# MAC-VO/MAC-VO

Measured on NVIDIA H100. Metric: stereo frames/sec @640x480, higher is better.
Workload: dtype f32

## Files before the change

### include/macvo_b200.h

```cpp
#ifndef MACVO_B200_H
#define MACVO_B200_H

#include <stddef.h>
#include <stdint.h>

#ifdef __cplusplus
extern "C" {
#endif

#define MACVO_OK 0
#define MACVO_E_ARG (-1)
#define MACVO_E_WORKSPACE (-2)
#define MACVO_E_UNSUPPORTED (-3)
#define MACVO_E_DRIVER (-4)

const char* macvo_b200_version(void);

#define MACVO_CORR_SIMT 0
#define MACVO_CORR_TC_3XF16 1
#define MACVO_CORR_TC_1XF16 2
#define MACVO_CORR_TC_TF32 3
#define MACVO_CORR_KMAJOR_INPUT 16
size_t macvo_corr_workspace_bytes(int batch, int dim, int n, int mode);
int macvo_corr_build(const float* fmap1, const float* fmap2, float* corr, int batch, int dim, int n, int mode,
// ... 88 lines not shown
                            const double* intr, double* pose_io, const macvo_pgo_params_t* params, double* stats,
                            void* const* exchange_bufs, int world, int rank, void* stream);

#define MACVO_PGO_ACC 55
#define MACVO_PGO_MAX_RANKS 8
int macvo_pgo_accumulate(const double* pos_Tw, const double* kp2_uv, const double* kp2_disp, const double* uv_cov,
                         const double* disp_cov, int k, const double* intr, const double* pose, double huber_delta,
                         double* acc, void* stream);

int macvo_layer_norm(const float* x, const float* weight, const float* bias, float* y, long long rows,
                     int channels, float eps, void* stream);
int macvo_add_layer_norm(const float* x, const float* resid, const float* weight, const float* bias, float* sum_out,
                         float* y, long long rows, int channels, float eps, void* stream);
int macvo_mlp_tc(const float* xn, const float* resid, const float* w1, const float* b1, const float* w2, const float* b2,
                 float* out, int rows, int channels, int hidden, void* stream);
int macvo_patch_tokens_tc(const float* x, const float* w0, const float* term, const float* w2, const float* b2,
                          const float* ln_w, const float* ln_b, float* out, long long rows, int in_channels, int channels,
                          int period, float eps, void* stream);
int macvo_patch_embed_conv1(const float* maps, const float* weight, const float* bias, float* out,
                            long long n_maps, int h, int w, int allow_tf32, void* stream);
int macvo_add_rows_relu(float* x, const float* term, long long rows, int period, int channels, void* stream);
int macvo_small_attention(const float* q, const float* k, const float* v, float* out, int batch, int nq, int nk,
                          int heads, int head_dim, int q_broadcast, int allow_tf32, void* stream);

int macvo_small_attention_ex(const float* q, const float* k, const float* v, float* out, int batch, int nq, int nk,
                             int heads, int head_dim, int q_broadcast, int allow_tf32, int ldq, int ldk, int ldv,
                             const float* q_add, const float* k_add, int add_period, void* stream);

int macvo_latent_pool(const float* tokens, const float* ut, const float* wv, const float* bv, float* out,
                      long long n_maps, int nk, void* stream);
// ... 76 lines not shown
```

### mac-vo_b200/csrc/mlp_tc.cu

```cuda
#include "tc_common.cuh"

namespace {

constexpr int MLP_C = 128, MLP_ROWS = 128, MLP_CHUNK = 64;
constexpr int XN_BYTES = MLP_ROWS * MLP_C * 4;
constexpr int XN_SUB = MLP_ROWS * 128;
constexpr int W1_BYTES = MLP_CHUNK * MLP_C * 4;
constexpr int W1_SUB = MLP_CHUNK * 128;
constexpr int W2_BYTES = MLP_C * MLP_CHUNK * 4;
constexpr int W2_SUB = MLP_C * 128;
constexpr int HID_WG_BYTES = 64 * MLP_CHUNK * 4;
constexpr int HID_SUB = 64 * 128;
constexpr int OFF_W1 = XN_BYTES, OFF_W2 = OFF_W1 + 2 * W1_BYTES, OFF_HID = OFF_W2 + 2 * W2_BYTES;
constexpr int OFF_BAR = OFF_HID + 2 * HID_WG_BYTES;
constexpr int MLP_SMEM = OFF_BAR + 128 + 1024;
static_assert(MLP_SMEM <= 227 * 1024, "shared memory budget");

constexpr uint32_t SW128_DESC_HI = (1024u >> 4) | (1u << 30);
__device__ __forceinline__ uint32_t sw128_lo(uint32_t smem_addr) { return ((smem_addr & 0x3FFFFu) >> 4) | (1u << 16); }
__device__ __forceinline__ uint64_t sw128_desc(uint32_t lo) { return ((uint64_t)SW128_DESC_HI << 32) | lo; }

__device__ __forceinline__ uint32_t to_tf32(float x) {
    uint32_t r;
    asm("cvt.rn.tf32.f32 %0, %1;" : "=r"(r) : "f"(x));
    return r;
}

constexpr int MLP_THREADS = TC_CONSUMER_THREADS + 128;

__global__ void __launch_bounds__(MLP_THREADS, 1)
mlp_tc_kernel(const __grid_constant__ CUtensorMap map_x, const __grid_constant__ CUtensorMap map_w1,
              const __grid_constant__ CUtensorMap map_w2, const float* __restrict__ b1, const float* __restrict__ b2,
              const float* __restrict__ resid, float* __restrict__ out, int m, int hd) {
    extern __shared__ uint8_t smem_raw[];
    uint8_t* smem = reinterpret_cast<uint8_t*>((reinterpret_cast<uintptr_t>(smem_raw) + 1023) & ~(uintptr_t)1023);
    const uint32_t s_base = smem_u32(smem);
    const uint32_t bar_x = s_base + OFF_BAR, bar_w1f = bar_x + 8, bar_w1e = bar_w1f + 16, bar_w2f = bar_w1e + 16,
                   bar_w2e = bar_w2f + 16;
    const int warp = threadIdx.x >> 5, lane = threadIdx.x & 31;
    const int m0 = blockIdx.x * MLP_ROWS, chunks = hd / MLP_CHUNK;

    if (threadIdx.x == 0) {
        mbar_init(bar_x, 1);
        for (int s = 0; s < 2; ++s) {
            mbar_init(bar_w1f + 8 * s, 1); mbar_init(bar_w1e + 8 * s, 2);
            mbar_init(bar_w2f + 8 * s, 1); mbar_init(bar_w2e + 8 * s, 2);
        }
        fence_barrier_init();
        prefetch_tmap(&map_x); prefetch_tmap(&map_w1); prefetch_tmap(&map_w2);
    }
    __syncthreads();

    if (warp >= TC_PRODUCER_WARP) {
        asm volatile("setmaxnreg.dec.sync.aligned.u32 40;");
        if (warp == TC_PRODUCER_WARP && elect_one()) {
            mbar_expect_tx(bar_x, XN_BYTES);
            for (int kc = 0; kc < 4; ++kc) tma_load_2d(s_base + kc * XN_SUB, &map_x, bar_x, 32 * kc, m0);
            for (int j = 0; j < chunks; ++j) {
                const int s = j & 1;
                const uint32_t parity = ((j >> 1) & 1) ^ 1;
                mbar_wait(bar_w1e + 8 * s, parity);
                mbar_expect_tx(bar_w1f + 8 * s, W1_BYTES);
                for (int kc = 0; kc < 4; ++kc)
                    tma_load_2d(s_base + OFF_W1 + s * W1_BYTES + kc * W1_SUB, &map_w1, bar_w1f + 8 * s, 32 * kc, j * MLP_CHUNK);
                mbar_wait(bar_w2e + 8 * s, parity);
                mbar_expect_tx(bar_w2f + 8 * s, W2_BYTES);
                for (int h = 0; h < 2; ++h)
                    tma_load_2d(s_base + OFF_W2 + s * W2_BYTES + h * W2_SUB, &map_w2, bar_w2f + 8 * s, j * MLP_CHUNK + 32 * h, 0);
            }
        }
        return;
    }
// ... 34 lines not shown
        if (leader) {
            mbar_arrive(bar_w1e + 8 * (j & 1));
            if (j > 0) mbar_arrive(bar_w2e + 8 * ((j - 1) & 1));
        }
        const float* bj = b1 + j * MLP_CHUNK;
#pragma unroll
        for (int i = 0; i < 32; i += 2) {
            const int r = fr + 8 * ((i >> 1) & 1), c = 8 * (i >> 2) + fc;
            const float2 bb = __ldg(reinterpret_cast<const float2*>(bj + c));
            const uint32_t v0 = to_tf32(gelu_erf(h[i] + bb.x)), v1 = to_tf32(gelu_erf(h[i + 1] + bb.y));
            const int cc = c & 31;
            const uint32_t addr = hid + (c >> 5) * HID_SUB + r * 128 + ((((cc >> 2) ^ (r & 7))) << 4) + (cc & 3) * 4;
            asm volatile("st.shared.v2.b32 [%0], {%1, %2};" ::"r"(addr), "r"(v0), "r"(v1) : "memory");
        }
        asm volatile("fence.proxy.async.shared::cta;" ::: "memory");
        if (wg == 0) asm volatile("bar.sync 2, 128;" ::: "memory");
        else asm volatile("bar.sync 3, 128;" ::: "memory");
        const int s = j & 1;
        mbar_wait(bar_w2f + 8 * s, (j >> 1) & 1);
        uint32_t hd_ = hid_d;
        asm volatile("" : "+r"(hd_));
        const uint32_t wb = hd_ - ((OFF_HID + wg * HID_WG_BYTES) >> 4) + ((OFF_W2 + s * W2_BYTES) >> 4);
        wgmma_fence();
#pragma unroll
        for (int hh = 0; hh < 2; ++hh) {
#pragma unroll
            for (int k = 0; k < 4; ++k)
                Wgmma<128>::tf32(acc, sw128_desc(hd_ + (hh * HID_SUB >> 4) + 2 * k), sw128_desc(wb + (hh * W2_SUB >> 4) + 2 * k),
                                 (j | hh | k) != 0);
        }
        wgmma_commit();
    };

    mbar_wait(bar_x, 0);
    {
        const int t = threadIdx.x & 127;
#pragma unroll
        for (int kc = 0; kc < 4; ++kc) {
#pragma unroll
            for (int u = 0; u < 4; ++u) {
                const uint32_t a = s_base + kc * XN_SUB + wg * 64 * 128 + (u * 128 + t) * 16;
                const float4 v = lds128(a);
                asm volatile("st.shared.v4.b32 [%0], {%1, %2, %3, %4};" ::"r"(a), "r"(to_tf32(v.x)), "r"(to_tf32(v.y)),
                             "r"(to_tf32(v.z)), "r"(to_tf32(v.w)) : "memory");
            }
        }
        asm volatile("fence.proxy.async.shared::cta;" ::: "memory");
        if (wg == 0) asm volatile("bar.sync 2, 128;" ::: "memory");
        else asm volatile("bar.sync 3, 128;" ::: "memory");
    }
    gemm1(h0, 0);
    for (int j = 0; j < chunks; j += 2) {
        chunk(h0, h1, j);
        chunk(h1, h0, j + 1);
    }
    wgmma_wait<0>();
    fence_acc(acc);

    const int row0 = m0 + wg * 64 + fr;
#pragma unroll
    for (int i = 0; i < 64; i += 2) {
        const int r = row0 + 8 * ((i >> 1) & 1), c = 8 * (i >> 2) + fc;
        if (r < m) {
            const float2 bb = __ldg(reinterpret_cast<const float2*>(b2 + c));
            const float2 x = __ldg(reinterpret_cast<const float2*>(resid + (long long)r * MLP_C + c));
            *reinterpret_cast<float2*>(out + (long long)r * MLP_C + c) = make_float2(x.x + (acc[i] + bb.x), x.y + (acc[i + 1] + bb.y));
        }
    }
}

}

int macvo_mlp_tc(const float* xn, const float* resid, const float* w1, const float* b1, const float* w2, const float* b2,
                 float* out, int rows, int channels, int hidden, void* stream) {
    if (!xn || !resid || !w1 || !b1 || !w2 || !b2 || !out || rows <= 0) return MACVO_E_ARG;
    if (channels != MLP_C || (hidden != 128 && hidden != 512)) return MACVO_E_UNSUPPORTED;
    for (const void* p : {(const void*)xn, (const void*)resid, (const void*)w1, (const void*)b1, (const void*)w2,
                          (const void*)b2, (const void*)out})
        if (reinterpret_cast<uintptr_t>(p) & 15) return MACVO_E_ARG;
    CUtensorMap m_x, m_w1, m_w2;
    bool ok = make_map_2d(&m_x, CU_TENSOR_MAP_DATA_TYPE_FLOAT32, 4, xn, MLP_C, rows, MLP_C * 4, 32, MLP_ROWS);
    ok = ok && make_map_2d(&m_w1, CU_TENSOR_MAP_DATA_TYPE_FLOAT32, 4, w1, MLP_C, hidden, MLP_C * 4, 32, MLP_CHUNK);
    ok = ok && make_map_2d(&m_w2, CU_TENSOR_MAP_DATA_TYPE_FLOAT32, 4, w2, hidden, MLP_C, (uint64_t)hidden * 4, 32, MLP_C);
    if (!ok) return MACVO_E_DRIVER;
    static bool configured = false;
    if (!configured) {
        MACVO_CUDA_TRY(cudaFuncSetAttribute(mlp_tc_kernel, cudaFuncAttributeMaxDynamicSharedMemorySize, MLP_SMEM));
        configured = true;
    }
    mlp_tc_kernel<<<ceil_div(rows, MLP_ROWS), MLP_THREADS, MLP_SMEM, as_stream(stream)>>>(m_x, m_w1, m_w2, b1, b2, resid, out,
                                                                                          rows, hidden);
    MACVO_LAUNCH_CHECK();
    return MACVO_OK;
}
```

### mac-vo_b200/flowformer_cov.py

```python
from __future__ import annotations

import math
import os
import zlib
from typing import Callable

import torch
import torch.nn.functional as F

Tensor = torch.Tensor

LATENT_TOKENS = 8
LATENT_DIM = 128
QUERY_DIM = 64
COST_INPUT_DIM = 64
VERT_C_DIM = 64
ENCODER_DEPTH = 3


def _svt_spec(prefix: str) -> list[tuple[str, tuple[int, ...], str]]:
    out: list[tuple[str, tuple[int, ...], str]] = []
    dims, heads, srs, patch, cin = (128, 256), (4, 8), (8, 4), (4, 2), (3, 128)
    for s, (C, sr, ps, ci) in enumerate(zip(dims, srs, patch, cin)):
        p = f"{prefix}.svt."
# ... 272 lines not shown
        return o.permute(0, 2, 1, 3).reshape(B, I, C)

    def _memo(self, key, fn):
        if key not in self._cache:
            self._cache[key] = fn()
        return self._cache[key]

    def svt(self, x: Tensor, prefix: str) -> Tensor:
        B = x.shape[0]
        for s, (heads, sr, ps) in enumerate(((4, 8, 4), (8, 4, 2))):
            p = f"{prefix}.svt."
            x = self._conv(x, p + f"patch_embeds.{s}.proj", stride=ps)
            C, H, W = x.shape[1:]
            x = self._ln(x.flatten(2).transpose(1, 2), p + f"patch_embeds.{s}.norm")
            b0, b1 = p + f"blocks.{s}.0.", p + f"blocks.{s}.1."
            x, xn = self._add_ln(x, self._svt_local_attn(self._ln(x, b0 + "norm1", 1e-6), (H, W), b0 + "attn.", heads), b0 + "norm2", 1e-6)
            x = self._mlp_residual(x, xn, b0 + "mlp.", "fc1", "fc2")
            t = x.transpose(1, 2).reshape(B, C, H, W)
            t = self._conv(t, p + f"pos_block.{s}.proj.0", padding=1, groups=C) + t
            x = t.flatten(2).transpose(1, 2)
            x, xn = self._add_ln(x, self._svt_global_attn(self._ln(x, b1 + "norm1", 1e-6), (H, W), b1 + "attn.", heads, sr), b1 + "norm2", 1e-6)
            x = self._mlp_residual(x, xn, b1 + "mlp.", "fc1", "fc2")
            x = x.reshape(B, H, W, C).permute(0, 3, 1, 2)
        return x

    def _mlp_residual(self, x: Tensor, xn: Tensor, p: str, fc1: str, fc2: str) -> Tensor:
        w1 = self.W[p + fc1 + ".weight"]
        if (self.mlp_tensor_cores and self._native(x) and torch.backends.cuda.matmul.allow_tf32 and x.shape[-1] == 128
                and w1.shape[0] in self._ops.MLP_TC_HIDDEN and x.is_contiguous() and xn.is_contiguous()):
            w1t, w2t = self._memo(("mlp_tc", p), lambda: (self._ops.round_tf32(w1), self._ops.round_tf32(self.W[p + fc2 + ".weight"])))
            return self._ops.mlp_tc(xn, x, w1t, self.W[p + fc1 + ".bias"], w2t, self.W[p + fc2 + ".bias"])
        return x + self._lin(F.gelu(self._lin(xn, p + fc1)), p + fc2)

    @staticmethod
    def _to_windows(x: Tensor, ws: int) -> tuple[Tensor, tuple[int, int, int, int]]:
        B, H, W, C = x.shape
        pr, pb = (ws - W % ws) % ws, (ws - H % ws) % ws
        x = F.pad(x, (0, 0, 0, pr, 0, pb))
        nh, nw = (H + pb) // ws, (W + pr) // ws
        x = x.reshape(B, nh, ws, nw, ws, C).transpose(2, 3).reshape(B * nh * nw, ws * ws, C)
        return x, (B, nh, nw, C)

    @staticmethod
    def _from_windows(x: Tensor, meta: tuple[int, int, int, int], ws: int, H: int, W: int) -> Tensor:
        B, nh, nw, C = meta
        x = x.reshape(B, nh, nw, ws, ws, C).transpose(2, 3).reshape(B, nh * ws, nw * ws, C)
        return x[:, :H, :W, :].reshape(B, H * W, C)

    def _svt_local_attn(self, x: Tensor, size, p: str, heads: int, ws: int = 7) -> Tensor:
        B, N, C = x.shape
        H, W = size
        xw, meta = self._to_windows(x.view(B, H, W, C), ws)
        wq, bq = self.W[p + "qkv.weight"], self.W[p + "qkv.bias"]
        q, k, v = (F.linear(xw, wq[i * C:(i + 1) * C], bq[i * C:(i + 1) * C]) for i in range(3))
        o = self._attn(q, k, v, heads)
        return self._lin(self._from_windows(o, meta, ws, H, W), p + "proj")

    def _svt_global_attn(self, x: Tensor, size, p: str, heads: int, sr: int) -> Tensor:
        B, N, C = x.shape
        q = self._lin(x, p + "q")
        t = self._conv(x.permute(0, 2, 1).reshape(B, C, *size), p + "sr", stride=sr)
        t = self._ln(t.reshape(B, C, -1).permute(0, 2, 1), p + "norm")
        wkv, bkv = self.W[p + "kv.weight"], self.W[p + "kv.bias"]
        o = self._attn(q, F.linear(t, wkv[:C], bkv[:C]), F.linear(t, wkv[C:], bkv[C:]), heads)
        return self._lin(o, p + "proj")

    def patch_embed(self, cost_maps: Tensor) -> Tensor:
        p = "memory_encoder.cost_perceiver_encoder.patch_embed."
        M, _, H2, W2 = cost_maps.shape
        if self._native(cost_maps) and (H2 + 7) // 8 * 8 * ((W2 + 7) // 8 * 8) <= 96 * 160:
            if torch.backends.cudnn.allow_tf32:
                x = self._ops.patch_embed_conv1(cost_maps, self.W[p + "proj.0.weight"], self.W[p + "proj.0.bias"], s2d=True)
                w2 = self._memo(("pe_w2_s2d", x.device), lambda: self._ops.space_to_depth_filter(self.W[p + "proj.2.weight"])
                                .contiguous(memory_format=torch.channels_last))
                x = torch.cudnn_convolution_relu(x, w2, self.W[p + "proj.2.bias"], (1, 1), (1, 1), (1, 1), 1)
            else:
                x = self._ops.patch_embed_conv1(cost_maps, self.W[p + "proj.0.weight"], self.W[p + "proj.0.bias"])
                x = self._conv_relu(x, p + "proj.2", stride=2, padding=2)
        else:
            x = F.pad(cost_maps, (0, (8 - W2 % 8) % 8, 0, (8 - H2 % 8) % 8))
# ... 17 lines not shown
        t = x.permute(0, 2, 3, 1).reshape(M, h * w, COST_INPUT_DIM)
        w2 = self.W[p + "ffn_with_coord.2.weight"][:, :, 0, 0]
        if native and torch.backends.cuda.matmul.allow_tf32:
            w0t, w2t = self._memo(("pe_tc", x.device), lambda: (self._ops.round_tf32(w0[:, :COST_INPUT_DIM, 0, 0]),
                                                                self._ops.round_tf32(w2)))
            return self._ops.patch_tokens_tc(t, w0t, term[0], w2t, self.W[p + "ffn_with_coord.2.bias"],
                                             self.W[p + "norm.weight"], self.W[p + "norm.bias"])
        t = F.linear(t, w0[:, :COST_INPUT_DIM, 0, 0])
        t = self._ops.add_rows_relu_(t, term[0]) if native else F.relu(t + term)
        t = F.linear(t, w2, self.W[p + "ffn_with_coord.2.bias"])
        return self._ln(t, p + "norm")

    def _latent_layer(self, x: Tensor, p: str) -> Tensor:
        y = self._ln(x, p + "norm1")
        a = self._attn(self._lin(y, p + "q"), self._lin(y, p + "k"), self._lin(y, p + "v"), 8)
        x, xn = self._add_ln(x, self._lin(a, p + "proj"), p + "norm2")
        return self._mlp_residual(x, xn, p, "ffn.0", "ffn.3")

    def _context_tokens(self, context: Tensor, p: str, reps: int) -> Tensor:
        b, _, H, W = context.shape
        c = self._lin(context.flatten(2).permute(0, 2, 1), p + "context_proj").view(b, H, W, -1)
        return c.repeat(reps, 1, 1, 1)

    def _vert_local_attn_native(self, x: Tensor, size, context: Tensor, p: str, ws: int, heads: int) -> Tensor:
        Bt, N, C = x.shape
        H, W = size
        b = context.shape[0]
        wq, wk = self.W[p + "q.weight"], self.W[p + "k.weight"]
        enc = self._memo(("win", ws, C + VERT_C_DIM, x.dtype, x.device), lambda: sine_embed(
            coords_grid(1, ws, ws, x.device, x.dtype).view(1, 2, -1).permute(0, 2, 1), C + VERT_C_DIM))
        cproj = self._lin(context.flatten(2).permute(0, 2, 1), p + "context_proj").view(b, H, W, -1)
        cw, meta = self._to_windows(cproj, ws)
        w_qk_c = torch.cat([wq[:, C:], wk[:, C:]], 0)
        w_qk = torch.cat([wq, wk], 0)
        b_qk = torch.cat([self.W[p + "q.bias"], self.W[p + "k.bias"]], 0)
        terms = F.linear(cw, w_qk_c) + F.linear(enc, w_qk, b_qk)
        q_add, k_add = terms[..., :C].contiguous(), terms[..., C:].contiguous()
        w_x = self._memo(("vloc_w", p), lambda: torch.cat([wq[:, :C], wk[:, :C], self.W[p + "v.weight"]], 0).contiguous())
        b_x = self._memo(("vloc_b", p), lambda: torch.cat([torch.zeros(2 * C, device=x.device, dtype=x.dtype), self.W[p + "v.bias"]], 0))
        xw, meta = self._to_windows(x.view(Bt, H, W, C), ws)
        qkv = F.linear(xw, w_x, b_x)
        o = self._ops.fused_qkv_attention(qkv, heads, q_add, k_add)
        return self._lin(self._from_windows(o, meta, ws, H, W), p + "proj")

    def _vert_local_attn(self, x: Tensor, size, context: Tensor, p: str, ws: int = 7, heads: int = 8) -> Tensor:
        if self._native(x) and (x.shape[-1] // heads) in (16, 32):
            return self._vert_local_attn_native(x, size, context, p, ws, heads)
        Bt, N, C = x.shape
        H, W = size
        ctx = self._context_tokens(context, p, Bt // context.shape[0])
        xg = x.view(Bt, H, W, C)
        xw, meta = self._to_windows(xg, ws)
        qkw, _ = self._to_windows(torch.cat([xg, ctx], dim=-1), ws)
        enc = self._memo(("win", ws, C + VERT_C_DIM, x.dtype, x.device), lambda: sine_embed(
            coords_grid(1, ws, ws, x.device, x.dtype).view(1, 2, -1).permute(0, 2, 1), C + VERT_C_DIM))
        qkw = qkw + enc
        o = self._attn(self._lin(qkw, p + "q"), self._lin(qkw, p + "k"), self._lin(xw, p + "v"), heads)
        return self._lin(self._from_windows(o, meta, ws, H, W), p + "proj")

    def _vert_global_attn_native(self, x: Tensor, size, context: Tensor, p: str, sr: int, heads: int) -> Tensor:
        Bt, N, C = x.shape
        H, W = size
        b = context.shape[0]
        Cq = C + VERT_C_DIM
        wq = self.W[p + "q.weight"]
        cproj = self._lin(context.flatten(2).permute(0, 2, 1), p + "context_proj")
        enc_full = self._memo(("full", H, W, Cq, x.dtype, x.device), lambda: sine_embed(
            coords_grid(1, H, W, x.device, x.dtype).view(1, 2, -1).permute(0, 2, 1), Cq))
        q_add = (F.linear(cproj, wq[:, C:]) + F.linear(enc_full, wq, self.W[p + "q.bias"])).contiguous()
        q = F.linear(x, wq[:, :C])
        xg = x.view(Bt, H, W, C).permute(0, 3, 1, 2)
        wsk = self.W[p + "sr_key.weight"]
        wk_x = self._memo(("vglob_wkx", p), lambda: wsk[:, :C].contiguous(memory_format=torch.channels_last))
        wk_c = self._memo(("vglob_wkc", p), lambda: wsk[:, C:].contiguous(memory_format=torch.channels_last))
        k_ctx = F.conv2d(cproj.view(b, H, W, -1).permute(0, 3, 1, 2), wk_c, self.W[p + "sr_key.bias"], stride=sr)
        k_in = F.conv2d(xg, wk_x, None, stride=sr).permute(0, 2, 3, 1)
        M = k_in.shape[1] * k_in.shape[2]
        k_in = (k_in.reshape(Bt // b, b, M, C) + k_ctx.permute(0, 2, 3, 1).reshape(1, b, M, C)).view(Bt, M, C)
        v_in = self._conv(xg, p + "sr_value", stride=sr).reshape(Bt, C, -1).permute(0, 2, 1)
        v_in, k_in = self._ln(v_in, p + "norm"), self._ln(k_in, p + "norm")
        enc_sub = self._memo(("sub", H // sr, W // sr, sr, C, x.dtype, x.device), lambda: sine_embed(
            coords_grid(1, H // sr, W // sr, x.device, x.dtype).view(1, 2, -1).permute(0, 2, 1) * sr, C))
        o = self._ops.attention_with_terms(q, self._lin(k_in + enc_sub, p + "k"), self._lin(v_in, p + "v"), heads, q_add)
        return self._lin(o, p + "proj")

    def _vert_global_attn(self, x: Tensor, size, context: Tensor, p: str, sr: int = 4, heads: int = 8) -> Tensor:
        if self._native(x) and size[0] % sr == 0 and size[1] % sr == 0 and (x.shape[-1] // heads) in (16, 32):
            return self._vert_global_attn_native(x, size, context, p, sr, heads)
        Bt, N, C = x.shape
        H, W = size
        ctx = self._context_tokens(context, p, Bt // context.shape[0])
        xg = x.view(Bt, H, W, C)
        qk = torch.cat([xg, ctx], dim=-1)
        pr, pb = (sr - W % sr) % sr, (sr - H % sr) % sr
        xg, qk = F.pad(xg, (0, 0, 0, pr, 0, pb)), F.pad(qk, (0, 0, 0, pr, 0, pb))
        Hp, Wp = H + pb, W + pr
        Cq = C + VERT_C_DIM
        enc_full = self._memo(("full", Hp, Wp, Cq, x.dtype, x.device), lambda: sine_embed(
            coords_grid(1, Hp, Wp, x.device, x.dtype).view(1, 2, -1).permute(0, 2, 1), Cq))
        q = self._lin(qk.reshape(Bt, Hp * Wp, Cq) + enc_full, p + "q")
        v_in = self._conv(xg.permute(0, 3, 1, 2), p + "sr_value", stride=sr).reshape(Bt, C, -1).permute(0, 2, 1)
        k_in = self._conv(qk.permute(0, 3, 1, 2), p + "sr_key", stride=sr).reshape(Bt, C, -1).permute(0, 2, 1)
        v_in, k_in = self._ln(v_in, p + "norm"), self._ln(k_in, p + "norm")
        enc_sub = self._memo(("sub", Hp // sr, Wp // sr, sr, C, x.dtype, x.device), lambda: sine_embed(
            coords_grid(1, Hp // sr, Wp // sr, x.device, x.dtype).view(1, 2, -1).permute(0, 2, 1) * sr, C))
        o = self._attn(q, self._lin(k_in + enc_sub, p + "k"), self._lin(v_in, p + "v"), heads)
        o = o.view(Bt, Hp, Wp, C)[:, :H, :W, :].reshape(Bt, N, C)
        return self._lin(o, p + "proj")

    def _vert_block(self, x: Tensor, size, context: Tensor, p: str, local: bool) -> Tensor:
        attn = self._vert_local_attn if local else self._vert_global_attn
        x, xn = self._add_ln(x, attn(self._ln(x, p + "norm1"), size, context, p + "attn."), p + "norm2")
        return self._mlp_residual(x, xn, p + "mlp.", "fc1", "fc2")

    def cost_perceiver(self, cost_volume: Tensor, context: Tensor) -> tuple[Tensor, Tensor]:
        c = "memory_encoder.cost_perceiver_encoder."
        B, heads, H1, W1, H2, W2 = cost_volume.shape
        assert heads == 1
        cost_maps = cost_volume.view(B * H1 * W1, 1, H2, W2)
        tokens = self.patch_embed(cost_maps)
        p = c + "input_layer."
        lat = self.W[c + "latent_tokens"]
        M = tokens.shape[0]
        q = self._lin(self._ln(lat, p + "norm1"), p + "q")
        if self._native(tokens) and torch.backends.cuda.matmul.allow_tf32 and LATENT_DIM == 128 and LATENT_TOKENS == 8:
            a = self._ops.latent_pool(tokens, q[0], self.W[p + "k.weight"], self.W[p + "v.weight"], self.W[p + "v.bias"])
        else:
            a = self._attn(q, self._lin(tokens, p + "k"), self._lin(tokens, p + "v"), 8)
# ... 361 lines not shown
```

### mac-vo_b200/ops.py

```python
from __future__ import annotations

import ctypes as C
import os
import threading

import torch

from .build import LIB_PATH

Tensor = torch.Tensor

CORR_SIMT, CORR_TC_3XF16, CORR_TC_1XF16, CORR_TC_TF32 = 0, 1, 2, 3
CORR_MODE_NAMES = {0: "simt", 1: "tc3", 2: "tc1", 3: "tf32"}
CORR_KMAJOR_INPUT = 16
PGO_ACC = 55

_lib = None
_lock = threading.Lock()
LAUNCHES = [0]


class MacvoB200Error(RuntimeError):
    pass

# ... 52 lines not shown
    "macvo_observe_pack": (C.c_int, [C.c_void_p, C.c_int, C.c_int] + [C.c_void_p] * 6 + [C.c_int] * 3 + [C.c_void_p] * 2
                           + [C.c_int] + [C.c_float] * 3 + [C.c_void_p] * 6 + [C.c_size_t, C.c_void_p]
                           + [C.POINTER(_ObserveExt)]),
    "macvo_pgo_exchange_bytes": (C.c_size_t, [C.c_int]),
    "macvo_p2p_alloc": (C.c_int, [C.c_size_t, C.POINTER(C.c_void_p), C.c_char_p]),
    "macvo_p2p_open": (C.c_int, [C.c_char_p, C.POINTER(C.c_void_p)]),
    "macvo_p2p_close": (C.c_int, [C.c_void_p]),
    "macvo_p2p_free": (C.c_int, [C.c_void_p]),
    "macvo_pgo_solve_sharded": (C.c_int, [C.c_void_p] * 5 + [C.c_int, C.c_void_p, C.c_int, C.c_int] + [C.c_void_p] * 2
                                + [C.POINTER(_PgoParams)] + [C.c_void_p] * 2 + [C.c_int, C.c_int, C.c_void_p]),
    "macvo_pgo_accumulate": (C.c_int, [C.c_void_p] * 5 + [C.c_int] + [C.c_void_p] * 2 + [C.c_double]
                             + [C.c_void_p] * 2),
    "macvo_layer_norm": (C.c_int, [C.c_void_p] * 4 + [C.c_longlong, C.c_int, C.c_float, C.c_void_p]),
    "macvo_add_layer_norm": (C.c_int, [C.c_void_p] * 6 + [C.c_longlong, C.c_int, C.c_float, C.c_void_p]),
    "macvo_mlp_tc": (C.c_int, [C.c_void_p] * 7 + [C.c_int] * 3 + [C.c_void_p]),
    "macvo_patch_tokens_tc": (C.c_int, [C.c_void_p] * 8 + [C.c_longlong, C.c_int, C.c_int, C.c_int, C.c_float, C.c_void_p]),
    "macvo_patch_embed_conv1": (C.c_int, [C.c_void_p] * 4 + [C.c_longlong, C.c_int, C.c_int, C.c_int, C.c_void_p]),
    "macvo_add_rows_relu": (C.c_int, [C.c_void_p] * 2 + [C.c_longlong, C.c_int, C.c_int, C.c_void_p]),
    "macvo_small_attention": (C.c_int, [C.c_void_p] * 4 + [C.c_int] * 7 + [C.c_void_p]),
    "macvo_small_attention_ex": (C.c_int, [C.c_void_p] * 4 + [C.c_int] * 10 + [C.c_void_p] * 2 + [C.c_int, C.c_void_p]),
    "macvo_latent_pool": (C.c_int, [C.c_void_p] * 5 + [C.c_longlong, C.c_int, C.c_void_p]),
    "macvo_decoder_token_blob_floats": (C.c_size_t, []),
    "macvo_decoder_token": (C.c_int, [C.c_void_p] * 6 + [C.c_int, C.c_int, C.c_float, C.c_void_p]),
    "macvo_decoder_token_rows": (C.c_int, [C.c_void_p] * 6 + [C.c_int] * 3 + [C.c_float, C.c_void_p]),
    "macvo_gru_input": (C.c_int, [C.c_void_p] * 7 + [C.c_longlong, C.c_void_p]),
    "macvo_gru_gates": (C.c_int, [C.c_void_p] * 5 + [C.c_longlong, C.c_void_p]),
    "macvo_gru_blend": (C.c_int, [C.c_void_p] * 5 + [C.c_longlong, C.c_void_p]),
    "macvo_softmax_rows_f16": (C.c_int, [C.c_void_p] * 2 + [C.c_longlong, C.c_int, C.c_void_p]),
    "macvo_convex_upsample": (C.c_int, [C.c_void_p] * 3 + [C.c_float] + [C.c_int] * 3 + [C.c_void_p]),
    "macvo_rows_count": (C.c_size_t, [C.c_int] * 4),
# ... 691 lines not shown
    w1, w2 = _dev(w1, torch.float32, "mlp_tc w1"), _dev(w2, torch.float32, "mlp_tc w2")
    b1, b2 = _dev(b1, torch.float32, "mlp_tc b1"), _dev(b2, torch.float32, "mlp_tc b2")
    c, hd = xn.shape[-1], w1.shape[0]
    if (c != 128 or hd not in MLP_TC_HIDDEN or xn.shape != resid.shape or tuple(w1.shape) != (hd, c)
            or tuple(w2.shape) != (c, hd) or b1.numel() != hd or b2.numel() != c):
        raise MacvoB200Error(f"mlp_tc: unsupported shapes xn {tuple(xn.shape)}, resid {tuple(resid.shape)}, "
                             f"w1 {tuple(w1.shape)}, w2 {tuple(w2.shape)}")
    out = torch.empty_like(resid)
    rc = load_library().macvo_mlp_tc(xn.data_ptr(), resid.data_ptr(), w1.data_ptr(), b1.data_ptr(), w2.data_ptr(),
                                      b2.data_ptr(), out.data_ptr(), xn.numel() // c, c, hd, _stream())
    _check(rc, "macvo_mlp_tc")
    LAUNCHES[0] += 1
    return out


def patch_tokens_tc(x: Tensor, w0: Tensor, term: Tensor, w2: Tensor, b2: Tensor, ln_w: Tensor, ln_b: Tensor,
                    eps: float = 1e-5) -> Tensor:
    x, term = _dev(x, torch.float32, "patch_tokens_tc x"), _dev(term, torch.float32, "patch_tokens_tc term")
    w0, w2 = _dev(w0, torch.float32, "patch_tokens_tc w0"), _dev(w2, torch.float32, "patch_tokens_tc w2")
    b2 = _dev(b2, torch.float32, "patch_tokens_tc b2")
    ln_w, ln_b = _dev(ln_w, torch.float32, "patch_tokens_tc ln_w"), _dev(ln_b, torch.float32, "patch_tokens_tc ln_b")
    cin, c = x.shape[-1], w0.shape[0]
    if (cin != 64 or c != 128 or tuple(w0.shape) != (c, cin) or tuple(w2.shape) != (c, c) or term.dim() != 2
            or term.shape[1] != c or term.shape[0] == 0 or any(t.numel() != c for t in (b2, ln_w, ln_b))):
        raise MacvoB200Error(f"patch_tokens_tc: unsupported shapes x {tuple(x.shape)}, w0 {tuple(w0.shape)}, "
                             f"term {tuple(term.shape)}, w2 {tuple(w2.shape)}")
    out = torch.empty(*x.shape[:-1], c, dtype=torch.float32, device=x.device)
    rc = load_library().macvo_patch_tokens_tc(x.data_ptr(), w0.data_ptr(), term.data_ptr(), w2.data_ptr(), b2.data_ptr(),
                                              ln_w.data_ptr(), ln_b.data_ptr(), out.data_ptr(), x.numel() // cin, cin, c,
                                              term.shape[0], float(eps), _stream())
# ... 469 lines not shown
```

Measured before the change: 47.51.

## Fuse attention output projection, residual add and LayerNorm into the TC MLP kernel

Adds a PROJ-templated variant of the TMA/wgmma MLP kernel. It first runs the attention output projection as a tf32 GEMM, adds the bias and residual, writes the sum out, then applies LayerNorm in shared memory before the existing fc1/GELU/fc2 pipeline. The projection weight and residual tile reuse the W1/W2 ring buffers, with a new mbarrier that holds the producer back until that data is consumed. Every transformer block calls this kernel, which removes a separate linear launch, the add-LN kernel and the intermediate global round trips. The cost is a serialized projection phase ahead of the MLP pipeline, plus an extra write and read-back of out.

New measurement: 48.31 (median of 6 runs). +1.7%, better.

```diff
diff --git a/include/macvo_b200.h b/include/macvo_b200.h
--- a/include/macvo_b200.h
+++ b/include/macvo_b200.h
@@ -126,6 +126,9 @@
                          float* y, long long rows, int channels, float eps, void* stream);
 int macvo_mlp_tc(const float* xn, const float* resid, const float* w1, const float* b1, const float* w2, const float* b2,
                  float* out, int rows, int channels, int hidden, void* stream);
+int macvo_attn_out_mlp_tc(const float* a, const float* resid, const float* w_proj, const float* b_proj, const float* ln_w,
+                          const float* ln_b, float eps, const float* w1, const float* b1, const float* w2, const float* b2,
+                          float* out, int rows, int channels, int hidden, void* stream);
 int macvo_patch_tokens_tc(const float* x, const float* w0, const float* term, const float* w2, const float* b2,
                           const float* ln_w, const float* ln_b, float* out, long long rows, int in_channels, int channels,
                           int period, float eps, void* stream);
diff --git a/mac-vo_b200/csrc/mlp_tc.cu b/mac-vo_b200/csrc/mlp_tc.cu
--- a/mac-vo_b200/csrc/mlp_tc.cu
+++ b/mac-vo_b200/csrc/mlp_tc.cu
@@ -1,4 +1,5 @@
 #include "tc_common.cuh"
+#include "layer_norm_row.cuh"
 
 namespace {
 
@@ -15,6 +16,9 @@
 constexpr int OFF_BAR = OFF_HID + 2 * HID_WG_BYTES;
 constexpr int MLP_SMEM = OFF_BAR + 128 + 1024;
 static_assert(MLP_SMEM <= 227 * 1024, "shared memory budget");
+constexpr int WP_SUB = MLP_C * 128;
+static_assert(4 * WP_SUB == 2 * W1_BYTES, "W_proj fills the W1 ring");
+static_assert(XN_BYTES == 2 * W2_BYTES, "the resid tile fills the W2 ring");
 
 constexpr uint32_t SW128_DESC_HI = (1024u >> 4) | (1u << 30);
 __device__ __forceinline__ uint32_t sw128_lo(uint32_t smem_addr) { return ((smem_addr & 0x3FFFFu) >> 4) | (1u << 16); }
@@ -28,15 +32,24 @@
 
 constexpr int MLP_THREADS = TC_CONSUMER_THREADS + 128;
 
+__device__ __forceinline__ void wg_sync(int wg) {
+    if (wg == 0) asm volatile("bar.sync 2, 128;" ::: "memory");
+    else asm volatile("bar.sync 3, 128;" ::: "memory");
+}
+
+template <bool PROJ>
 __global__ void __launch_bounds__(MLP_THREADS, 1)
 mlp_tc_kernel(const __grid_constant__ CUtensorMap map_x, const __grid_constant__ CUtensorMap map_w1,
-              const __grid_constant__ CUtensorMap map_w2, const float* __restrict__ b1, const float* __restrict__ b2,
+              const __grid_constant__ CUtensorMap map_w2, const __grid_constant__ CUtensorMap map_wp,
+              const __grid_constant__ CUtensorMap map_r,
+              const float* __restrict__ b1, const float* __restrict__ b2, const float* __restrict__ b_proj,
+              const float* __restrict__ ln_w, const float* __restrict__ ln_b, float eps,
               const float* __restrict__ resid, float* __restrict__ out, int m, int hd) {
     extern __shared__ uint8_t smem_raw[];
     uint8_t* smem = reinterpret_cast<uint8_t*>((reinterpret_cast<uintptr_t>(smem_raw) + 1023) & ~(uintptr_t)1023);
     const uint32_t s_base = smem_u32(smem);
     const uint32_t bar_x = s_base + OFF_BAR, bar_w1f = bar_x + 8, bar_w1e = bar_w1f + 16, bar_w2f = bar_w1e + 16,
-                   bar_w2e = bar_w2f + 16;
+                   bar_w2e = bar_w2f + 16, bar_pd = bar_w2e + 16;
     const int warp = threadIdx.x >> 5, lane = threadIdx.x & 31;
     const int m0 = blockIdx.x * MLP_ROWS, chunks = hd / MLP_CHUNK;
 
@@ -46,16 +59,23 @@
             mbar_init(bar_w1f + 8 * s, 1); mbar_init(bar_w1e + 8 * s, 2);
             mbar_init(bar_w2f + 8 * s, 1); mbar_init(bar_w2e + 8 * s, 2);
         }
+        if (PROJ) mbar_init(bar_pd, 2);
         fence_barrier_init();
         prefetch_tmap(&map_x); prefetch_tmap(&map_w1); prefetch_tmap(&map_w2);
+        if (PROJ) { prefetch_tmap(&map_wp); prefetch_tmap(&map_r); }
     }
     __syncthreads();
 
     if (warp >= TC_PRODUCER_WARP) {
         asm volatile("setmaxnreg.dec.sync.aligned.u32 40;");
         if (warp == TC_PRODUCER_WARP && elect_one()) {
-            mbar_expect_tx(bar_x, XN_BYTES);
+            mbar_expect_tx(bar_x, PROJ ? 2 * XN_BYTES + 4 * WP_SUB : XN_BYTES);
             for (int kc = 0; kc < 4; ++kc) tma_load_2d(s_base + kc * XN_SUB, &map_x, bar_x, 32 * kc, m0);
+            if (PROJ) {
+                for (int kc = 0; kc < 4; ++kc) tma_load_2d(s_base + OFF_W1 + kc * WP_SUB, &map_wp, bar_x, 32 * kc, 0);
+                for (int kc = 0; kc < 4; ++kc) tma_load_2d(s_base + OFF_W2 + kc * XN_SUB, &map_r, bar_x, 32 * kc, m0);
+                mbar_wait(bar_pd, 0);
+            }
             for (int j = 0; j < chunks; ++j) {
                 const int s = j & 1;
                 const uint32_t parity = ((j >> 1) & 1) ^ 1;
@@ -120,8 +140,7 @@
             asm volatile("st.shared.v2.b32 [%0], {%1, %2};" ::"r"(addr), "r"(v0), "r"(v1) : "memory");
         }
         asm volatile("fence.proxy.async.shared::cta;" ::: "memory");
-        if (wg == 0) asm volatile("bar.sync 2, 128;" ::: "memory");
-        else asm volatile("bar.sync 3, 128;" ::: "memory");
+        wg_sync(wg);
         const int s = j & 1;
         mbar_wait(bar_w2f + 8 * s, (j >> 1) & 1);
         uint32_t hd_ = hid_d;
@@ -152,8 +171,52 @@
             }
         }
         asm volatile("fence.proxy.async.shared::cta;" ::: "memory");
-        if (wg == 0) asm volatile("bar.sync 2, 128;" ::: "memory");
-        else asm volatile("bar.sync 3, 128;" ::: "memory");
+        wg_sync(wg);
+    }
+    if (PROJ) {
+        {
+            uint32_t ad = xa, wd = sw128_lo(s_base + OFF_W1);
+            asm volatile("" : "+r"(ad), "+r"(wd));
+            wgmma_fence();
+#pragma unroll
+            for (int kc = 0; kc < 4; ++kc) {
+#pragma unroll
+                for (int k = 0; k < 4; ++k)
+                    Wgmma<128>::tf32(acc, sw128_desc(ad + (kc * XN_SUB >> 4) + 2 * k), sw128_desc(wd + (kc * WP_SUB >> 4) + 2 * k),
+                                     (kc | k) != 0);
+            }
+            wgmma_commit();
+            wgmma_wait<0>();
+            fence_acc(acc);
+        }
+        wg_sync(wg);
+        const int row0 = m0 + wg * 64 + fr;
+#pragma unroll
+        for (int i = 0; i < 64; i += 2) {
+            const int r = fr + 8 * ((i >> 1) & 1), c = 8 * (i >> 2) + fc, gr = row0 + 8 * ((i >> 1) & 1);
+            const int cc = c & 31, tr = wg * 64 + r;
+            const uint32_t off = (c >> 5) * XN_SUB + tr * 128 + (((cc >> 2) ^ (tr & 7)) << 4) + (cc & 3) * 4;
+            const float2 bb = __ldg(reinterpret_cast<const float2*>(b_proj + c));
+            float2 rr;
+            asm volatile("ld.shared.v2.f32 {%0, %1}, [%2];" : "=f"(rr.x), "=f"(rr.y) : "r"(s_base + OFF_W2 + off) : "memory");
+            const float2 x = make_float2(rr.x + (acc[i] + bb.x), rr.y + (acc[i + 1] + bb.y));
+            if (gr < m) *reinterpret_cast<float2*>(out + (long long)gr * MLP_C + c) = x;
+            sts64(s_base + off, x.x, x.y);
+        }
+        wg_sync(wg);
+        if (leader) mbar_arrive(bar_pd);
+#pragma unroll
+        for (int j = 0; j < 16; ++j) {
+            const int tr = wg * 64 + (warp & 3) * 16 + j;
+            const uint32_t addr = s_base + (lane >> 3) * XN_SUB + tr * 128 + (((lane & 7) ^ (tr & 7)) << 4);
+            const float4 x4 = lds128(addr);
+            float v[4] = {x4.x, x4.y, x4.z, x4.w};
+            layer_norm_row<4>(v, ln_w, ln_b, eps, lane);
+            asm volatile("st.shared.v4.b32 [%0], {%1, %2, %3, %4};" ::"r"(addr), "r"(to_tf32(v[0])), "r"(to_tf32(v[1])),
+                         "r"(to_tf32(v[2])), "r"(to_tf32(v[3])) : "memory");
+        }
+        asm volatile("fence.proxy.async.shared::cta;" ::: "memory");
+        wg_sync(wg);
     }
     gemm1(h0, 0);
     for (int j = 0; j < chunks; j += 2) {
@@ -169,10 +232,38 @@
         const int r = row0 + 8 * ((i >> 1) & 1), c = 8 * (i >> 2) + fc;
         if (r < m) {
             const float2 bb = __ldg(reinterpret_cast<const float2*>(b2 + c));
-            const float2 x = __ldg(reinterpret_cast<const float2*>(resid + (long long)r * MLP_C + c));
-            *reinterpret_cast<float2*>(out + (long long)r * MLP_C + c) = make_float2(x.x + (acc[i] + bb.x), x.y + (acc[i + 1] + bb.y));
-        }
-    }
+            float2* o = reinterpret_cast<float2*>(out + (long long)r * MLP_C + c);
+            const float2 x = PROJ ? *o : __ldg(reinterpret_cast<const float2*>(resid + (long long)r * MLP_C + c));
+            *o = make_float2(x.x + (acc[i] + bb.x), x.y + (acc[i + 1] + bb.y));
+        }
+    }
+}
+
+int mlp_tc_launch(const float* x, const float* resid, const float* w1, const float* b1, const float* w2, const float* b2,
+                  const float* w_proj, const float* b_proj, const float* ln_w, const float* ln_b, float eps, float* out,
+                  int rows, int hidden, void* stream) {
+    CUtensorMap m_x, m_w1, m_w2, m_wp, m_r;
+    bool ok = make_map_2d(&m_x, CU_TENSOR_MAP_DATA_TYPE_FLOAT32, 4, x, MLP_C, rows, MLP_C * 4, 32, MLP_ROWS);
+    ok = ok && make_map_2d(&m_w1, CU_TENSOR_MAP_DATA_TYPE_FLOAT32, 4, w1, MLP_C, hidden, MLP_C * 4, 32, MLP_CHUNK);
+    ok = ok && make_map_2d(&m_w2, CU_TENSOR_MAP_DATA_TYPE_FLOAT32, 4, w2, hidden, MLP_C, (uint64_t)hidden * 4, 32, MLP_C);
+    m_wp = m_w1;
+    m_r = m_x;
+    if (w_proj) {
+        ok = ok && make_map_2d(&m_wp, CU_TENSOR_MAP_DATA_TYPE_FLOAT32, 4, w_proj, MLP_C, MLP_C, MLP_C * 4, 32, MLP_C);
+        ok = ok && make_map_2d(&m_r, CU_TENSOR_MAP_DATA_TYPE_FLOAT32, 4, resid, MLP_C, rows, MLP_C * 4, 32, MLP_ROWS);
+    }
+    if (!ok) return MACVO_E_DRIVER;
+    static bool configured = false;
+    if (!configured) {
+        MACVO_CUDA_TRY(cudaFuncSetAttribute(mlp_tc_kernel<false>, cudaFuncAttributeMaxDynamicSharedMemorySize, MLP_SMEM));
+        MACVO_CUDA_TRY(cudaFuncSetAttribute(mlp_tc_kernel<true>, cudaFuncAttributeMaxDynamicSharedMemorySize, MLP_SMEM));
+        configured = true;
+    }
+    auto kernel = w_proj ? mlp_tc_kernel<true> : mlp_tc_kernel<false>;
+    kernel<<<ceil_div(rows, MLP_ROWS), MLP_THREADS, MLP_SMEM, as_stream(stream)>>>(m_x, m_w1, m_w2, m_wp, m_r, b1, b2, b_proj, ln_w,
+                                                                                   ln_b, eps, resid, out, rows, hidden);
+    MACVO_LAUNCH_CHECK();
+    return MACVO_OK;
 }
 
 }
@@ -184,18 +275,17 @@
     for (const void* p : {(const void*)xn, (const void*)resid, (const void*)w1, (const void*)b1, (const void*)w2,
                           (const void*)b2, (const void*)out})
         if (reinterpret_cast<uintptr_t>(p) & 15) return MACVO_E_ARG;
-    CUtensorMap m_x, m_w1, m_w2;
-    bool ok = make_map_2d(&m_x, CU_TENSOR_MAP_DATA_TYPE_FLOAT32, 4, xn, MLP_C, rows, MLP_C * 4, 32, MLP_ROWS);
-    ok = ok && make_map_2d(&m_w1, CU_TENSOR_MAP_DATA_TYPE_FLOAT32, 4, w1, MLP_C, hidden, MLP_C * 4, 32, MLP_CHUNK);
-    ok = ok && make_map_2d(&m_w2, CU_TENSOR_MAP_DATA_TYPE_FLOAT32, 4, w2, hidden, MLP_C, (uint64_t)hidden * 4, 32, MLP_C);
-    if (!ok) return MACVO_E_DRIVER;
-    static bool configured = false;
-    if (!configured) {
-        MACVO_CUDA_TRY(cudaFuncSetAttribute(mlp_tc_kernel, cudaFuncAttributeMaxDynamicSharedMemorySize, MLP_SMEM));
-        configured = true;
-    }
-    mlp_tc_kernel<<<ceil_div(rows, MLP_ROWS), MLP_THREADS, MLP_SMEM, as_stream(stream)>>>(m_x, m_w1, m_w2, b1, b2, resid, out,
-                                                                                          rows, hidden);
-    MACVO_LAUNCH_CHECK();
-    return MACVO_OK;
-}
+    return mlp_tc_launch(xn, resid, w1, b1, w2, b2, nullptr, nullptr, nullptr, nullptr, 0.f, out, rows, hidden, stream);
+}
+
+int macvo_attn_out_mlp_tc(const float* a, const float* resid, const float* w_proj, const float* b_proj, const float* ln_w,
+                          const float* ln_b, float eps, const float* w1, const float* b1, const float* w2, const float* b2,
+                          float* out, int rows, int channels, int hidden, void* stream) {
+    if (!a || !resid || !w_proj || !b_proj || !ln_w || !ln_b || !w1 || !b1 || !w2 || !b2 || !out || rows <= 0)
+        return MACVO_E_ARG;
+    if (channels != MLP_C || (hidden != 128 && hidden != 512)) return MACVO_E_UNSUPPORTED;
+    for (const void* p : {(const void*)a, (const void*)resid, (const void*)w_proj, (const void*)b_proj, (const void*)ln_w,
+                          (const void*)ln_b, (const void*)w1, (const void*)b1, (const void*)w2, (const void*)b2, (const void*)out})
+        if (reinterpret_cast<uintptr_t>(p) & 15) return MACVO_E_ARG;
+    return mlp_tc_launch(a, resid, w1, b1, w2, b2, w_proj, b_proj, ln_w, ln_b, eps, out, rows, hidden, stream);
+}
diff --git a/mac-vo_b200/flowformer_cov.py b/mac-vo_b200/flowformer_cov.py
--- a/mac-vo_b200/flowformer_cov.py
+++ b/mac-vo_b200/flowformer_cov.py
@@ -310,23 +310,37 @@
             C, H, W = x.shape[1:]
             x = self._ln(x.flatten(2).transpose(1, 2), p + f"patch_embeds.{s}.norm")
             b0, b1 = p + f"blocks.{s}.0.", p + f"blocks.{s}.1."
-            x, xn = self._add_ln(x, self._svt_local_attn(self._ln(x, b0 + "norm1", 1e-6), (H, W), b0 + "attn.", heads), b0 + "norm2", 1e-6)
-            x = self._mlp_residual(x, xn, b0 + "mlp.", "fc1", "fc2")
+            a = self._svt_local_attn(self._ln(x, b0 + "norm1", 1e-6), (H, W), b0 + "attn.", heads)
+            x = self._attn_out_mlp(x, a, b0 + "attn.proj", b0 + "norm2", b0 + "mlp.", "fc1", "fc2", 1e-6)
             t = x.transpose(1, 2).reshape(B, C, H, W)
             t = self._conv(t, p + f"pos_block.{s}.proj.0", padding=1, groups=C) + t
             x = t.flatten(2).transpose(1, 2)
-            x, xn = self._add_ln(x, self._svt_global_attn(self._ln(x, b1 + "norm1", 1e-6), (H, W), b1 + "attn.", heads, sr), b1 + "norm2", 1e-6)
-            x = self._mlp_residual(x, xn, b1 + "mlp.", "fc1", "fc2")
+            a = self._svt_global_attn(self._ln(x, b1 + "norm1", 1e-6), (H, W), b1 + "attn.", heads, sr)
+            x = self._attn_out_mlp(x, a, b1 + "attn.proj", b1 + "norm2", b1 + "mlp.", "fc1", "fc2", 1e-6)
             x = x.reshape(B, H, W, C).permute(0, 3, 1, 2)
         return x
 
-    def _mlp_residual(self, x: Tensor, xn: Tensor, p: str, fc1: str, fc2: str) -> Tensor:
+    def _mlp_tc_weights(self, x: Tensor, p: str, fc1: str, fc2: str) -> tuple[Tensor, Tensor] | None:
         w1 = self.W[p + fc1 + ".weight"]
         if (self.mlp_tensor_cores and self._native(x) and torch.backends.cuda.matmul.allow_tf32 and x.shape[-1] == 128
-                and w1.shape[0] in self._ops.MLP_TC_HIDDEN and x.is_contiguous() and xn.is_contiguous()):
-            w1t, w2t = self._memo(("mlp_tc", p), lambda: (self._ops.round_tf32(w1), self._ops.round_tf32(self.W[p + fc2 + ".weight"])))
-            return self._ops.mlp_tc(xn, x, w1t, self.W[p + fc1 + ".bias"], w2t, self.W[p + fc2 + ".bias"])
+                and w1.shape[0] in self._ops.MLP_TC_HIDDEN and x.is_contiguous()):
+            return self._memo(("mlp_tc", p), lambda: (self._ops.round_tf32(w1), self._ops.round_tf32(self.W[p + fc2 + ".weight"])))
+        return None
+
+    def _mlp_residual(self, x: Tensor, xn: Tensor, p: str, fc1: str, fc2: str) -> Tensor:
+        w = self._mlp_tc_weights(x, p, fc1, fc2)
+        if w is not None and xn.is_contiguous():
+            return self._ops.mlp_tc(xn, x, w[0], self.W[p + fc1 + ".bias"], w[1], self.W[p + fc2 + ".bias"])
         return x + self._lin(F.gelu(self._lin(xn, p + fc1)), p + fc2)
+
+    def _attn_out_mlp(self, x: Tensor, a: Tensor, proj: str, norm2: str, p: str, fc1: str, fc2: str, eps: float = 1e-5) -> Tensor:
+        w = self._mlp_tc_weights(x, p, fc1, fc2)
+        if w is not None and a.shape == x.shape:
+            wp = self._memo(("mlp_tc", proj), lambda: self._ops.round_tf32(self.W[proj + ".weight"]))
+            return self._ops.attn_out_mlp_tc(a, x, wp, self.W[proj + ".bias"], self.W[norm2 + ".weight"], self.W[norm2 + ".bias"],
+                                             w[0], self.W[p + fc1 + ".bias"], w[1], self.W[p + fc2 + ".bias"], eps)
+        x, xn = self._add_ln(x, self._lin(a, proj), norm2, eps)
+        return self._mlp_residual(x, xn, p, fc1, fc2)
 
     @staticmethod
     def _to_windows(x: Tensor, ws: int) -> tuple[Tensor, tuple[int, int, int, int]]:
@@ -350,7 +364,7 @@
         wq, bq = self.W[p + "qkv.weight"], self.W[p + "qkv.bias"]
         q, k, v = (F.linear(xw, wq[i * C:(i + 1) * C], bq[i * C:(i + 1) * C]) for i in range(3))
         o = self._attn(q, k, v, heads)
-        return self._lin(self._from_windows(o, meta, ws, H, W), p + "proj")
+        return self._from_windows(o, meta, ws, H, W)
 
     def _svt_global_attn(self, x: Tensor, size, p: str, heads: int, sr: int) -> Tensor:
         B, N, C = x.shape
@@ -358,8 +372,7 @@
         t = self._conv(x.permute(0, 2, 1).reshape(B, C, *size), p + "sr", stride=sr)
         t = self._ln(t.reshape(B, C, -1).permute(0, 2, 1), p + "norm")
         wkv, bkv = self.W[p + "kv.weight"], self.W[p + "kv.bias"]
-        o = self._attn(q, F.linear(t, wkv[:C], bkv[:C]), F.linear(t, wkv[C:], bkv[C:]), heads)
-        return self._lin(o, p + "proj")
+        return self._attn(q, F.linear(t, wkv[:C], bkv[:C]), F.linear(t, wkv[C:], bkv[C:]), heads)
 
     def patch_embed(self, cost_maps: Tensor) -> Tensor:
         p = "memory_encoder.cost_perceiver_encoder.patch_embed."
@@ -407,8 +420,7 @@
     def _latent_layer(self, x: Tensor, p: str) -> Tensor:
         y = self._ln(x, p + "norm1")
         a = self._attn(self._lin(y, p + "q"), self._lin(y, p + "k"), self._lin(y, p + "v"), 8)
-        x, xn = self._add_ln(x, self._lin(a, p + "proj"), p + "norm2")
-        return self._mlp_residual(x, xn, p, "ffn.0", "ffn.3")
+        return self._attn_out_mlp(x, a, p + "proj", p + "norm2", p, "ffn.0", "ffn.3")
 
     def _context_tokens(self, context: Tensor, p: str, reps: int) -> Tensor:
         b, _, H, W = context.shape
@@ -434,7 +446,7 @@
         xw, meta = self._to_windows(x.view(Bt, H, W, C), ws)
         qkv = F.linear(xw, w_x, b_x)
         o = self._ops.fused_qkv_attention(qkv, heads, q_add, k_add)
-        return self._lin(self._from_windows(o, meta, ws, H, W), p + "proj")
+        return self._from_windows(o, meta, ws, H, W)
 
     def _vert_local_attn(self, x: Tensor, size, context: Tensor, p: str, ws: int = 7, heads: int = 8) -> Tensor:
         if self._native(x) and (x.shape[-1] // heads) in (16, 32):
@@ -449,7 +461,7 @@
             coords_grid(1, ws, ws, x.device, x.dtype).view(1, 2, -1).permute(0, 2, 1), C + VERT_C_DIM))
         qkw = qkw + enc
         o = self._attn(self._lin(qkw, p + "q"), self._lin(qkw, p + "k"), self._lin(xw, p + "v"), heads)
-        return self._lin(self._from_windows(o, meta, ws, H, W), p + "proj")
+        return self._from_windows(o, meta, ws, H, W)
 
     def _vert_global_attn_native(self, x: Tensor, size, context: Tensor, p: str, sr: int, heads: int) -> Tensor:
         Bt, N, C = x.shape
@@ -474,8 +486,7 @@
         v_in, k_in = self._ln(v_in, p + "norm"), self._ln(k_in, p + "norm")
         enc_sub = self._memo(("sub", H // sr, W // sr, sr, C, x.dtype, x.device), lambda: sine_embed(
             coords_grid(1, H // sr, W // sr, x.device, x.dtype).view(1, 2, -1).permute(0, 2, 1) * sr, C))
-        o = self._ops.attention_with_terms(q, self._lin(k_in + enc_sub, p + "k"), self._lin(v_in, p + "v"), heads, q_add)
-        return self._lin(o, p + "proj")
+        return self._ops.attention_with_terms(q, self._lin(k_in + enc_sub, p + "k"), self._lin(v_in, p + "v"), heads, q_add)
 
     def _vert_global_attn(self, x: Tensor, size, context: Tensor, p: str, sr: int = 4, heads: int = 8) -> Tensor:
         if self._native(x) and size[0] % sr == 0 and size[1] % sr == 0 and (x.shape[-1] // heads) in (16, 32):
@@ -498,13 +509,12 @@
         enc_sub = self._memo(("sub", Hp // sr, Wp // sr, sr, C, x.dtype, x.device), lambda: sine_embed(
             coords_grid(1, Hp // sr, Wp // sr, x.device, x.dtype).view(1, 2, -1).permute(0, 2, 1) * sr, C))
         o = self._attn(q, self._lin(k_in + enc_sub, p + "k"), self._lin(v_in, p + "v"), heads)
-        o = o.view(Bt, Hp, Wp, C)[:, :H, :W, :].reshape(Bt, N, C)
-        return self._lin(o, p + "proj")
+        return o.view(Bt, Hp, Wp, C)[:, :H, :W, :].reshape(Bt, N, C)
 
     def _vert_block(self, x: Tensor, size, context: Tensor, p: str, local: bool) -> Tensor:
         attn = self._vert_local_attn if local else self._vert_global_attn
-        x, xn = self._add_ln(x, attn(self._ln(x, p + "norm1"), size, context, p + "attn."), p + "norm2")
-        return self._mlp_residual(x, xn, p + "mlp.", "fc1", "fc2")
+        a = attn(self._ln(x, p + "norm1"), size, context, p + "attn.")
+        return self._attn_out_mlp(x, a, p + "attn.proj", p + "norm2", p + "mlp.", "fc1", "fc2")
 
     def cost_perceiver(self, cost_volume: Tensor, context: Tensor) -> tuple[Tensor, Tensor]:
         c = "memory_encoder.cost_perceiver_encoder."
diff --git a/mac-vo_b200/ops.py b/mac-vo_b200/ops.py
--- a/mac-vo_b200/ops.py
+++ b/mac-vo_b200/ops.py
@@ -90,6 +90,7 @@
     "macvo_layer_norm": (C.c_int, [C.c_void_p] * 4 + [C.c_longlong, C.c_int, C.c_float, C.c_void_p]),
     "macvo_add_layer_norm": (C.c_int, [C.c_void_p] * 6 + [C.c_longlong, C.c_int, C.c_float, C.c_void_p]),
     "macvo_mlp_tc": (C.c_int, [C.c_void_p] * 7 + [C.c_int] * 3 + [C.c_void_p]),
+    "macvo_attn_out_mlp_tc": (C.c_int, [C.c_void_p] * 6 + [C.c_float] + [C.c_void_p] * 5 + [C.c_int] * 3 + [C.c_void_p]),
     "macvo_patch_tokens_tc": (C.c_int, [C.c_void_p] * 8 + [C.c_longlong, C.c_int, C.c_int, C.c_int, C.c_float, C.c_void_p]),
     "macvo_patch_embed_conv1": (C.c_int, [C.c_void_p] * 4 + [C.c_longlong, C.c_int, C.c_int, C.c_int, C.c_void_p]),
     "macvo_add_rows_relu": (C.c_int, [C.c_void_p] * 2 + [C.c_longlong, C.c_int, C.c_int, C.c_void_p]),
@@ -811,6 +812,28 @@
     return out
 
 
+def attn_out_mlp_tc(a: Tensor, resid: Tensor, w_proj: Tensor, b_proj: Tensor, ln_w: Tensor, ln_b: Tensor, w1: Tensor,
+                    b1: Tensor, w2: Tensor, b2: Tensor, eps: float = 1e-5) -> Tensor:
+    a, resid = _dev(a, torch.float32, "attn_out_mlp_tc a"), _dev(resid, torch.float32, "attn_out_mlp_tc resid")
+    w_proj, b_proj = _dev(w_proj, torch.float32, "attn_out_mlp_tc w_proj"), _dev(b_proj, torch.float32, "attn_out_mlp_tc b_proj")
+    ln_w, ln_b = _dev(ln_w, torch.float32, "attn_out_mlp_tc ln_w"), _dev(ln_b, torch.float32, "attn_out_mlp_tc ln_b")
+    w1, w2 = _dev(w1, torch.float32, "attn_out_mlp_tc w1"), _dev(w2, torch.float32, "attn_out_mlp_tc w2")
+    b1, b2 = _dev(b1, torch.float32, "attn_out_mlp_tc b1"), _dev(b2, torch.float32, "attn_out_mlp_tc b2")
+    c, hd = a.shape[-1], w1.shape[0]
+    if (c != 128 or hd not in MLP_TC_HIDDEN or a.shape != resid.shape or tuple(w_proj.shape) != (c, c)
+            or tuple(w1.shape) != (hd, c) or tuple(w2.shape) != (c, hd) or b1.numel() != hd
+            or any(t.numel() != c for t in (b_proj, ln_w, ln_b, b2))):
+        raise MacvoB200Error(f"attn_out_mlp_tc: unsupported shapes a {tuple(a.shape)}, resid {tuple(resid.shape)}, "
+                             f"w_proj {tuple(w_proj.shape)}, w1 {tuple(w1.shape)}, w2 {tuple(w2.shape)}")
+    out = torch.empty_like(resid)
+    rc = load_library().macvo_attn_out_mlp_tc(a.data_ptr(), resid.data_ptr(), w_proj.data_ptr(), b_proj.data_ptr(),
+                                              ln_w.data_ptr(), ln_b.data_ptr(), float(eps), w1.data_ptr(), b1.data_ptr(),
+                                              w2.data_ptr(), b2.data_ptr(), out.data_ptr(), a.numel() // c, c, hd, _stream())
+    _check(rc, "macvo_attn_out_mlp_tc")
+    LAUNCHES[0] += 1
+    return out
+
+
 def patch_tokens_tc(x: Tensor, w0: Tensor, term: Tensor, w2: Tensor, b2: Tensor, ln_w: Tensor, ln_b: Tensor,
                     eps: float = 1e-5) -> Tensor:
     x, term = _dev(x, torch.float32, "patch_tokens_tc x"), _dev(term, torch.float32, "patch_tokens_tc term")
```
